# seqan/sahara

Hardware: AMD Instinct MI355X
Metric: reads/s at k=2 edit, 10M×100bp vs 3Gbp index; achieved HBM GB/s (higher is better)
Workload: dtype u32; 1 GPU; C3: k=2 lev, 10000000x100bp reads (+RC) per GPU vs 3 Gbp 24-record index, h2-k2; reads_per_gpu=10000000, read_len=100, errors=2, ref_len=3000000000, records=24, generator=h2-k2, searches=3, parallelism=replicated-index x1 (query shards), hits_total=25990613, build_id=362c7fb006402490

## Files before the change

sahara_amd/csrc/pass.cpp:

```cpp
#include <algorithm>
#include <cstdlib>
#include <chrono>
#include <thread>

#include <sys/prctl.h>

#include "ctx.h"

namespace sahara {

DeviceIndex& partOf(Ctx* c, uint32_t p) { return p == 0 ? c->I : c->more.at(p - 1); }

void run(Ctx* c, bool count) {
    if (c->more.empty()) return runOne(c, count);
    if (c->rounds.size() > 1) throw Error("a pass of several rounds needs a single-part index");
    const ScopeExit routeBack([c, route = c->sk.route] { c->sk.route = route; });
    c->sk.route = HitRoute::Device;
    sahara_stats T{};
    uint64_t total = 0;
    const auto t0 = std::chrono::steady_clock::now();
    for (uint32_t p = 0; p <= c->more.size(); ++p) {
        if (p) std::swap(c->I, c->more[p - 1]);
        {
            const ScopeExit partBack([c, p] {
// ... 54 lines not shown
    S.stage_ms = c->stageMs;
    c->stats = S;
}

const sahara_hit* Ctx::wholeHits() {
    if (outStale) {
        if (out.cap < nout) out.growKeeping(nout, out.cap, st);
        uint64_t b0 = 0;
        for (size_t b = 0; b < batchEnd.size(); b0 = batchEnd[b], ++b)
            if (batchDirect[b])
                launchExpandRecs(outRecs.ptr + b0, batchEnd[b] - b0, batchQ0[b], I.dRecStarts.ptr,
                                 (uint32_t)I.recStarts.size(), out.ptr + b0, st);
        SH_HIP(hipStreamSynchronize(st));
        outStale = false;
    }
    return out.ptr;
}

void initWorkCaps(Ctx* c, uint64_t maxBatch, const PassKnobs& k) {
    if (c->hitCap == 0) c->hitCap = k.hitCap ? k.hitCap : firstWorkCap(maxBatch);
    if (c->taskCap == 0) c->taskCap = k.taskCap ? k.taskCap : firstWorkCap(maxBatch);
}

void reserveSlot(Ctx* c, Ctx::Slot& sl) {
    sl.hits.reserve((size_t)c->hitCap + 1);
    sl.rank.reserve((size_t)c->hitCap + 1);
    sl.tasks.reserve((size_t)c->taskCap);
}

void reserveLocate(Ctx* c, uint64_t maxBatch, uint64_t nslots) {
    c->qoff.reserve(maxBatch + 1);
    c->big.reserve(maxBatch);
    c->huge.reserve(maxBatch);
    for (uint64_t i = 0; i < nslots; ++i) c->slot[i].qcnt.reserve(maxBatch + 1);
}

void growCap(uint32_t& cap, uint32_t seen) {
    const uint64_t want = (uint64_t)seen + seen / 4 + 1024;
    if (want >= (1ull << 32) - 2) throw Error("a work buffer would exceed 2^32 entries in one batch");
    cap = std::max<uint32_t>(cap, (uint32_t)want);
}

static void waitSleepy(hipEvent_t e, uint32_t pollUs) {
    if (!pollUs) {
        SH_HIP(hipEventSynchronize(e));
        return;
    }
    for (;;) {
        const hipError_t r = hipEventQuery(e);
        if (r == hipSuccess) return;
        if (r != hipErrorNotReady) SH_HIP(r);
        std::this_thread::sleep_for(std::chrono::microseconds(pollUs));
    }
}

static PassPlan makePlan(Ctx* c, bool count, bool redo) {
    PassPlan P;
    P.k = readPassKnobs(c->verify);
    const PassKnobs& k = P.k;
    const bool serial = P.serial = redo || !k.pipeline;
    P.count = count;
    P.rounds = (uint32_t)c->rounds.size();
    const WorstRound worst = worstRound(c->rounds);
    if (worst.nsearch != c->nsearch || worst.maxErr != c->maxErr) throw Error("staged rounds do not match their plan");
    const uint32_t sigma = c->I.sigma;
    P.fmLds = fmLdsBytes(c->nsearch, c->m, k.fmLdsDepth);
    const int fullBpc = searchBlocksPerCU(sigma, c->edit, P.fmLds);
    int bpc = fullBpc;
    P.maxBatch = maxBatchOf(k.batch, c->sk.streaming, c->nsearch, c->sk.route == HitRoute::Records);
    const uint64_t batchesHere = (c->npat + P.maxBatch - 1) / P.maxBatch;
    if (!serial && batchesHere > 1 && c->verify) bpc = 1;
    if (k.fmBpc) bpc = (int)std::max<long>(1, std::min<long>(fullBpc, *k.fmBpc));
    P.blocks = (uint32_t)(c->numCU * bpc);
    P.firstBlocks = k.fmBpc ? P.blocks : (uint32_t)(c->numCU * fullBpc);
    P.stackLevels = P.stackCap = fmStackCap(c->maxErr, sigma);

    P.tx = textGeometry(c->m, c->maxErr, c->patBlocks, c->nsearch);
    const bool textFits = text3Blocks(c->I.n) * 16 <= 0xFFFFFF00ull &&
                          P.maxBatch * c->patBlocks * 16 <= 0xFFFFFF00ull;
    P.textShape = textShapeOf(P.tx.winBlocks, c->patBlocks, P.tx.exactWindow);
    auto textAlone = [&] { return textBlocksPerCU(sigma, c->edit, count, P.textShape, P.tx.lds); };
    int tbpc = c->verify && c->m <= 2047 && P.tx.lds <= 160 * 1024 && textFits ? textAlone() : 0;
    if (!serial && batchesHere > 1) tbpc = std::min(tbpc, 3);
    if (k.textBpc && tbpc > 0) tbpc = (int)std::max<long>(1, std::min<long>(textAlone(), *k.textBpc));
    if (k.dump)
        std::fprintf(stderr, "text geometry: shape %d lds %zu blocks/CU %d (alone %d) serial %d\n", P.textShape, P.tx.lds,
                     tbpc, textAlone(), (int)serial);
    P.textBpc = tbpc;
    P.textBlocks = (uint32_t)(c->numCU * std::max(tbpc, 1));
    P.split = tbpc > 0 ? k.split : 0u;
    P.toText = P.split >= 1 && k.seedTasks ? 1u : 0u;
    const bool chunkSeeds = c->sk.streaming && !serial && P.split && k.chunkSeeds;
    P.early = !serial && P.split && (batchesHere > 1 || chunkSeeds) && P.rounds == 1;
    P.chunked0 = P.early && chunkSeeds;
    P.sleepy = c->sk.streaming && !serial;
    P.probe = count && k.dump;
    P.bstart = batchStarts(c->npat, P.maxBatch, k.rampHead, k.rampTail, serial);
    return P;
}

static SearchArgs searchArgs(Ctx* c, const PassPlan& P, Ctx::Slot& sl, uint64_t b, uint32_t r) {
    const uint64_t q0 = P.bstart[b];
    const Ctx::Round& R = c->rounds[r];
    SearchArgs a{};
    a.occF = c->I.occF.ptr;
    a.occR = c->I.occR.ptr;
    for (int i = 0; i < 8; ++i) a.C[i] = (uint32_t)c->I.C[i];
    a.n = (uint32_t)c->I.n;
    a.pats = c->pats.ptr + q0 * c->patWords;
    a.patWords = c->patWords;
    a.m = c->m;
    a.nsearch = R.nsearch;
    a.nitems = (uint32_t)((P.bstart[b + 1] - q0) * R.nsearch);
    a.seeds = sl.seeds.ptr;
    a.seedItem = sl.seedItem.ptr;
    a.seedCount = sl.small.ptr + kSwSeedCount;
    a.scheme = c->scheme.ptr + R.schemeAt;
    a.work = sl.queues.ptr + kQueueSeeds;
    a.hitCount = sl.small.ptr + kSwHitCount;
    a.flags = sl.small.ptr + kSwFlags;
    a.filled = sl.small.ptr + kSwFilled;
    a.taskCount = sl.small.ptr + kSwTaskCount;
    a.stack = c->stack.ptr;
    a.stackCap = P.stackCap;
    a.stackLevels = P.stackLevels;
    a.stealAt = P.k.fmStealAt;
    a.hits = sl.hits.ptr;
    a.hitCap = c->hitCap;
    a.counters = c->counters.ptr;
    a.tasks = sl.tasks.ptr;
    a.taskCap = c->taskCap;
    a.split = P.split;
    a.ldsDepth = P.k.fmLdsDepth;
    a.qcnt = sl.qcnt.ptr;
    a.rank = sl.rank.ptr;
    return a;
}

static SeedArgs seedArgs(Ctx* c, const PassPlan& P, Ctx::Slot& sl, uint64_t b, uint32_t r) {
    const Ctx::Round& R = c->rounds[r];
    SeedArgs sd{};
    sd.pats = c->pats.ptr + P.bstart[b] * c->patWords;
    sd.patWords = c->patWords;
    sd.nsearch = R.nsearch;
    sd.nitems = (uint32_t)((P.bstart[b + 1] - P.bstart[b]) * R.nsearch);
    sd.n = (uint32_t)c->I.n;
    sd.kmer = c->verify && c->I.kmerK ? c->I.kmer.ptr : nullptr;
    sd.kmerK = c->I.kmerK;
    sd.kmerPos = c->I.kmerPos && P.k.kmerPos ? 1u : 0u;
    sd.kmerStart = c->kmerStart.ptr + R.kmerAt;
    sd.seeds = sl.seeds.ptr;
    sd.seedItem = sl.seedItem.ptr;
    sd.seedCount = sl.small.ptr + kSwSeedCount;
    sd.m = c->m;
    sd.toText = P.toText;
    sd.tasks = sl.tasks.ptr;
    sd.taskCap = c->taskCap;
    sd.taskCount = sl.small.ptr + kSwTaskCount;
    sd.flags = sl.small.ptr + kSwFlags;
    sd.counters = P.count ? c->counters.ptr : nullptr;
    sd.skip = r ? sl.qcnt.ptr : nullptr;
    return sd;
}

static TextBatchArgs textArgs(Ctx* c, const PassPlan& P, Ctx::Slot& sl, uint64_t b, uint32_t r) {
    const uint64_t q0 = P.bstart[b];
    const Ctx::Round& R = c->rounds[r];
    TextBatchArgs t{};
    t.sa = c->I.saFull.ptr;
    t.text3 = c->I.text3.ptr;
    t.pats3 = c->pats3.ptr + q0 * c->patBlocks;
    t.patBlocks = c->patBlocks;
    t.text3Bytes = (uint32_t)std::min<uint64_t>(text3Blocks(c->I.n) * 16, 0xFFFFFF00ull);
    t.pats3Bytes = (uint32_t)std::min<uint64_t>((P.bstart[b + 1] - q0) * c->patBlocks * 16, 0xFFFFFF00ull);
    t.m = c->m;
    t.nsearch = R.nsearch;
    t.table = reinterpret_cast<const uint2*>(c->cover.ptr + R.coverAt);
    t.tasks = sl.tasks.ptr;
    t.taskCount = sl.small.ptr + kSwTaskCount;
    t.taskBegin = r ? sl.small.ptr + kSwRoundTasks : nullptr;
    t.taskCap = c->taskCap;
    t.work = sl.queues.ptr + kQueueSeedTasks;
    t.hits = sl.hits.ptr;
    t.hitCap = c->hitCap;
    t.hitCount = sl.small.ptr + kSwHitCount;
    t.filled = sl.small.ptr + kSwFilled;
    t.flags = sl.small.ptr + kSwFlags;
    t.counters = c->counters.ptr;
    t.winBlocks = P.tx.winBlocks;
    t.exactWindow = P.tx.exactWindow ? 1u : 0u;
    t.stackCap = P.tx.textStack;
    t.tableWords = P.tx.tableWords;
    t.steps = P.k.textSteps;
    t.refillAt = P.k.refillAt;
    t.stealAt = P.k.stealAt;
    t.qcnt = sl.qcnt.ptr;
    t.rank = sl.rank.ptr;
    t.probe = P.probe ? 1u : 0u;
    t.isFirst = b == 0 && r == 0 ? 1u : 0u;
    return t;
}

enum : uint32_t { kLocFlags = 2, kLocSegCounts = 4 };

static LocateArgs locateArgs(Ctx* c, Ctx::Slot& sl, uint64_t nhits) {
    LocateArgs la{};
    la.hits = sl.hits.ptr;
    la.nhits = nhits;
    la.qoff = c->qoff.ptr;
    la.rank = sl.rank.ptr;
    la.occF = c->I.occF.ptr;
    for (int i = 0; i < 8; ++i) la.C[i] = (uint32_t)c->I.C[i];
    la.samples = c->I.samples.ptr;
    la.rate = c->I.rate;
    la.keys = c->k0.ptr;
    la.flags = c->small.ptr + kLocFlags;
    la.counters = c->counters.ptr + kCtLfSteps;
    la.sa = c->I.saFull.ptr;
    la.useSA = c->locateSA ? 1u : 0u;
    return la;
}

struct Pass {
    Ctx* c;
    const PassPlan& P;
    sahara_stats& S;
    bool& overflow;
    hipStream_t sA, sB, sC, sD;
    uint32_t seenTask = 0, seenHit = 0;

    Ctx::Slot& slotOf(uint64_t b) const { return c->slot[b % Ctx::kSlots]; }

    void resetSlot(Ctx::Slot& sl, hipStream_t s) {
        SH_HIP(hipMemsetAsync(sl.small.ptr, 0, kSlotWords * sizeof(uint32_t), s));
        SH_HIP(hipMemsetAsync(sl.queues.ptr, 0, kQueuesWords * sizeof(uint32_t), s));
        SH_HIP(hipEventRecord(sl.free, s));
    }
    void freeSlot(Ctx::Slot& sl, hipStream_t s) { SH_HIP(hipEventRecord(sl.free, s)); }

    void seedTasksDone(Ctx::Slot& sl) {
        SH_HIP(hipMemcpyAsync(sl.small.ptr + kSwSeedTasks, sl.small.ptr + kSwTaskCount, 4, hipMemcpyDeviceToDevice, sD));
    }

    struct RoundEv {
        hipEvent_t fmStart, seedDone, fmBegin, fmDone, textStart, textDone;
    };
    RoundEv eventsOf(Ctx::Slot& sl, uint32_t r) const {
        if (r + 1 == P.rounds) return {sl.fmStart, sl.seedDone, sl.fmBegin, sl.fmDone, sl.textStart, sl.textDone};
        Ctx::Slot::RoundEvents& e = sl.earlier[r];
        return {e.fmStart, e.seedDone, e.fmBegin, e.fmDone, e.textStart, e.textDone};
    }

    void issueFM(uint64_t b, uint32_t r) {
        Ctx::Slot& sl = slotOf(b);
        const std::vector<uint64_t>& bstart = P.bstart;
        const RoundEv ev = eventsOf(sl, r);
        const uint32_t nitems = (uint32_t)((bstart[b + 1] - bstart[b]) * c->rounds[r].nsearch);
        if (r == 0) {
            reserveSlot(c, sl);
            SH_HIP(hipStreamWaitEvent(sA, sl.free, 0));
            const uint32_t most = (uint32_t)((bstart[b + 1] - bstart[b]) * c->nsearch);
            sl.seeds.reserve(most);
            sl.seedItem.reserve(most);
        }
        const SearchArgs a = searchArgs(c, P, sl, b, r);
        SeedArgs sd = seedArgs(c, P, sl, b, r);
        if (r == 0) {
            SH_HIP(hipStreamWaitEvent(sD, sl.free, 0));
        } else {
            SH_HIP(hipStreamWaitEvent(sD, eventsOf(sl, r - 1).textDone, 0));
            launchRoundReset(sl.small.ptr, sl.queues.ptr, sD);
        }
        auto seeds = [&](uint32_t i0, uint32_t i1) {
            sd.itemBegin = i0;
            sd.nitems = i1;
            launchSeeds(sd, c->I.sigma, std::max<uint32_t>(1, std::min<uint32_t>((i1 - i0 + 1023) / 1024, (uint32_t)c->numCU * 8)), sD);
// ... 359 lines not shown
```

sahara_amd/csrc/search.hip:

```cpp

#include <hip/hip_runtime.h>

#include <cstring>
#include <type_traits>

#include <rocprim/rocprim.hpp>

#include "search.h"

namespace sahara {
namespace {

#if defined(__HIP_DEVICE_COMPILE__)
#define GLOB(T, p) ((__attribute__((address_space(1))) T*)(p))
#else
#define GLOB(T, p) ((T*)(p))
#endif
typedef uint32_t U32x4 __attribute__((ext_vector_type(4)));
__device__ __forceinline__ uint4 loadGlobal4(const uint4* p) {
    const U32x4 v = *GLOB(const U32x4, p);
    return make_uint4(v.x, v.y, v.z, v.w);
}

__device__ __forceinline__ uint32_t pairSwap(uint32_t v) {
// ... 445 lines not shown
            lo = right ? cur.y : cur.x;
            hi = lo + cur.z;
            needA = matchOK || misOK || delOK;
            needB = needA && (hi >> 6) != (lo >> 6);
        }

        const uint64_t ownA = (uint64_t)(right ? a.occR : a.occF) + (uint64_t)(lo >> 6) * 64u;
        const uint64_t ownB = (uint64_t)(right ? a.occR : a.occF) + (uint64_t)(hi >> 6) * 64u;
        uint32_t ca[5], cb[5];
        uint64_t pa[3], pb[3];
        fetchLinePair(ownA, needA, odd, ca, pa);
        fetchLinePair(ownB, needB, odd, cb, pb);

        if (have) {
            if (COUNT) ++cNodes;
            uint32_t occ[SIGMA], fx[SIGMA], fy[SIGMA];
#pragma unroll
            for (int c = 0; c < SIGMA; ++c) occ[c] = fx[c] = fy[c] = 0;
            if (needA) {
                if (!needB) {
#pragma unroll
                    for (int i = 0; i < 5; ++i) cb[i] = ca[i];
                    pb[0] = pa[0]; pb[1] = pa[1]; pb[2] = pa[2];
                }
                if (COUNT) { ++cRank; cLines += needB ? 2 : 1; }
                const uint64_t ml = lowMask(lo & 63u), mh = lowMask(hi & 63u);
                uint32_t sum = 0, base[SIGMA];
#pragma unroll
                for (int c = 1; c < SIGMA; ++c) {
                    const uint32_t rl = ca[c - 1] + (uint32_t)__popcll(symMask(pa, c) & ml);
                    const uint32_t rh = cb[c - 1] + (uint32_t)__popcll(symMask(pb, c) & mh);
                    occ[c] = rh - rl;
                    base[c] = a.C[c] + rl;
                    sum += occ[c];
                }
                uint32_t acc = (right ? cur.x : cur.y) + (cur.z - sum);
#pragma unroll
                for (int c = 1; c < SIGMA; ++c) {
                    fx[c] = right ? acc : base[c];
                    fy[c] = right ? base[c] : acc;
                    acc += occ[c];
                }
            }
            const uint32_t dl = metaDelta(cur.w);
            auto mk = [&](int c, uint32_t kind) -> uint4 {
                uint32_t f = 0, g = 0, o = 0;
#pragma unroll
                for (int s = 1; s < SIGMA; ++s)
                    if (s == c) { f = fx[s]; g = fy[s]; o = occ[s]; }
                return make_uint4(f, g, o, childMeta(pos, e, lastL, lastR, right, dl, kind));
            };
            auto push = [&](const uint4& v) {
                if (sp - bot < a.stackCap) {
                    stackPut(sp, v);
                    ++sp;
                } else {
                    atomicOr(a.flags, kFlagStack);
                }
            };
            const uint4 ins = make_uint4(cur.x, cur.y, cur.z, childMeta(pos, e, lastL, lastR, right, dl, 3));
            uint4 next = make_uint4(0, 0, 0, 0);
            have = expandChildren<SIGMA>(occ, cq, matchOK, misOK, delOK, insOK, ins, mk, push, next);
            cur = next;
        }
    }
    hitSlots.close(lane, a.hits, a.hitCap);
    taskSlots.close(lane, a.tasks, a.taskCap);
    if (filled) atomicAdd(a.filled, filled);
    if (COUNT) {
        atomicAdd(a.counters + kCtNodes, (unsigned long long)cNodes);
        atomicAdd(a.counters + kCtRankNodes, (unsigned long long)cRank);
        atomicAdd(a.counters + kCtExtLines, (unsigned long long)cLines);
        atomicAdd(a.counters + kCtTextTasks, (unsigned long long)cTasks);
        if (cIter) atomicAdd(a.counters + kCtFmIter, (unsigned long long)cIter);
    }
}




constexpr uint32_t kRun = 32;
constexpr uint32_t kRunMask = 0xFFFFFFFFu;
constexpr uint32_t kChain = 25;
__device__ __forceinline__ uint32_t onesR(uint32_t n) {
    return n >= kRun ? kRunMask : (1u << n) - 1u;
}
__device__ __forceinline__ uint32_t beyondR(uint32_t n) { return kRunMask & ~onesR(n); }
__device__ __forceinline__ uint32_t run7(uint32_t m) {
    const uint32_t m2 = m & (m >> 1), m4 = m2 & (m2 >> 2);
    return m4 & (m2 >> 4) & (m >> 6);
}
struct Planes { uint32_t b0, b1, b2; };
__device__ __forceinline__ uint32_t eqm(const Planes& p, const Planes& t) {
    return ~((p.b0 ^ t.b0) | (p.b1 ^ t.b1) | (p.b2 ^ t.b2));
}
__device__ __forceinline__ Planes shr1(const Planes& p) { return {p.b0 >> 1, p.b1 >> 1, p.b2 >> 1}; }
__device__ __forceinline__ Planes shr2(const Planes& p) { return {p.b0 >> 2, p.b1 >> 2, p.b2 >> 2}; }
__device__ __forceinline__ uint32_t read32(const uint32_t* A, int o, uint32_t b) {
    const int i = o >> 5;
    return __builtin_amdgcn_alignbit(A[(3 * i + 3 + (int)b) * 256], A[(3 * i + (int)b) * 256], (uint32_t)o & 31u);
}
__device__ __forceinline__ Planes chain32(const uint32_t* A, uint32_t o, bool fwd) {
    const int off = (int)o - (fwd ? 0 : 32);
    Planes r;
    uint32_t v[3];
#pragma unroll
    for (uint32_t b = 0; b < 3; ++b) {
        const uint32_t w = read32(A, off, b);
        v[b] = fwd ? w : __builtin_bitreverse32(w);
    }
    r.b0 = v[0]; r.b1 = v[1]; r.b2 = v[2];
    return r;
}

__device__ __forceinline__ __amdgpu_buffer_rsrc_t bufferOf(const void* base, uint32_t bytes) {
    return __builtin_amdgcn_make_buffer_rsrc(const_cast<void*>(base), (short)0, (int)bytes, 0x00020000);
}
constexpr uint32_t kBufOOB = 0xFFFFFFFFu;

__device__ __forceinline__ void copyBlocks(uint32_t* DA, __amdgpu_buffer_rsrc_t RA, uint32_t offA, uint32_t na,
                                           uint32_t* DB, __amdgpu_buffer_rsrc_t RB, uint32_t offB, uint32_t nb) {
    const uint32_t n = max(na, nb);
    for (uint32_t c = 0; c < n; c += 8) {
        decltype(__builtin_amdgcn_raw_buffer_load_b128(RA, 0u, 0, 0)) va[8], vb[8];
#pragma unroll
        for (uint32_t i = 0; i < 8; ++i) {
            const uint32_t j = c + i;
            va[i] = __builtin_amdgcn_raw_buffer_load_b128(RA, j < na ? offA + 16u * j : kBufOOB, 0, 0);
            vb[i] = __builtin_amdgcn_raw_buffer_load_b128(RB, j < nb ? offB + 16u * j : kBufOOB, 0, 0);
        }
#pragma unroll
        for (uint32_t i = 0; i < 8; ++i) {
            const uint32_t j = c + i;
            if (j < na) { uint32_t* D = DA + 3u * j * 256u; D[0] = va[i][0]; D[256] = va[i][1]; D[512] = va[i][2]; }
            if (j < nb) { uint32_t* D = DB + 3u * j * 256u; D[0] = vb[i][0]; D[256] = vb[i][1]; D[512] = vb[i][2]; }
        }
    }
}

__device__ __forceinline__ void copyBlocksShifted(uint32_t* DA, __amdgpu_buffer_rsrc_t RA, uint32_t offA, uint32_t sh,
                                                  uint32_t na, uint32_t* DB, __amdgpu_buffer_rsrc_t RB, uint32_t offB,
                                                  uint32_t nb) {
    decltype(__builtin_amdgcn_raw_buffer_load_b128(RA, 0u, 0, 0)) va[8], vb[8];
#pragma unroll
    for (uint32_t j = 0; j < 8; ++j) {
        va[j] = __builtin_amdgcn_raw_buffer_load_b128(RA, j <= na ? offA + 16u * j : kBufOOB, 0, 0);
        vb[j] = __builtin_amdgcn_raw_buffer_load_b128(RB, j < nb ? offB + 16u * j : kBufOOB, 0, 0);
    }
#pragma unroll
    for (uint32_t j = 0; j < 7; ++j)
        if (j < na) {
            uint32_t* D = DA + 3u * j * 256u;
            D[0] = __builtin_amdgcn_alignbit(va[j + 1][0], va[j][0], sh);
            D[256] = __builtin_amdgcn_alignbit(va[j + 1][1], va[j][1], sh);
            D[512] = __builtin_amdgcn_alignbit(va[j + 1][2], va[j][2], sh);
        }
#pragma unroll
    for (uint32_t j = 0; j < 8; ++j)
        if (j < nb) { uint32_t* D = DB + 3u * j * 256u; D[0] = vb[j][0]; D[256] = vb[j][1]; D[512] = vb[j][2]; }
}

struct TextShape { uint32_t win, pat; bool exact; };
__host__ __device__ constexpr TextShape textShape(int shape) {
    return shape == 1 ? TextShape{4, 4, true} : shape == 2 ? TextShape{9, 8, false} : TextShape{0, 0, false};
}


template <int SIGMA, bool EDIT, bool COUNT, int SHAPE = 0>
__global__ __launch_bounds__(256) void kSearchTextBatch(TextBatchArgs a) {
    extern __shared__ uint32_t lds[];
    uint2* SC = reinterpret_cast<uint2*>(lds);
    uint32_t* slot = lds + a.tableWords;
    for (uint32_t i = threadIdx.x; i < a.nsearch * a.m; i += blockDim.x) SC[i] = a.table[i];
    __syncthreads();
// ... 125 lines not shown
            const uint32_t nI = (uint32_t)__popcll(I), nD = (uint32_t)__popcll(D);
            if (nI >= a.stealAt && nD) {
                const uint32_t n = min(nI, nD);
                const uint32_t r = (uint32_t)__popcll(I & ltMask);
                uint32_t donor = 0, rr = r;
                uint64_t dm = D;
#pragma unroll
                for (uint32_t w = 32; w; w >>= 1) {
                    const uint32_t c = (uint32_t)__popcll(dm & ((1ull << w) - 1ull));
                    if (rr >= c) { rr -= c; dm >>= w; donor += w; }
                }
                const bool takes = thief && r < n;
                donor = takes ? donor : lane;
                const uint32_t dPid = __shfl(pid, donor), dWb = __shfl(wb, donor), dBase = __shfl(sBase, donor);
                const uint32_t dTid = (threadIdx.x & ~63u) | donor;
                if (takes) {
                    const uint32_t* src = slot + dTid;
                    uint32_t* dst = slot + threadIdx.x;
                    for (uint32_t k = 0; k < 3u * (winBlocks + patBlocks); ++k) dst[k * 256u] = src[k * 256u];
                    const uint2 node = reinterpret_cast<const uint2*>(slot + 3u * (winBlocks + patBlocks) * 256u)[dTid];
                    cur = node;
                    pid = dPid;
                    wb = dWb;
                    sBase = dBase;
                    have = true;
                    if (COUNT) ++cSteal;
                }
                __builtin_amdgcn_fence(__ATOMIC_ACQ_REL, "wavefront");
                __builtin_amdgcn_wave_barrier();
                const bool gives = ((D >> lane) & 1ull) && (uint32_t)__popcll(D & ltMask) < n;
                if (gives) {
                    for (uint32_t d = 1; d < sp; ++d) stackPut(d - 1u, stackGet(d));
                    --sp;
                }
            }
        }
        if (!__any(have || sp > 0 || (!exhausted && (!qDone || haveNext || qNext < qEnd)))) break;
        if (kProbe && a.probe) {
            if (qDone && lane == 0 && wDrain[threadIdx.x >> 6] == 0) wDrain[threadIdx.x >> 6] = wall_clock64();
            const uint32_t act = (uint32_t)__popcll(__ballot(have || sp > 0));
            if (qDone) { ++pIterPost; pActPost += act; } else { ++pIterPre; pActPre += act; }
            pw1 = wall_clock64();
        }
        if (COUNT) {
            const uint64_t act = __ballot(have || sp > 0);
            if (lane == 0) { ++tIter; tActive += (uint64_t)__popcll(act); tRefill += refill ? 1u : 0u; }
            const uint64_t t1 = clock64();
            cyRefill += t1 - t0;
            t0 = t1;
        }

        bool leaf = false;
        uint32_t leafStart = 0, leafE = 0;
        for (uint32_t step = 0; step < a.steps; ++step) {
            const bool pop = !have && !leaf && sp > 0;
            const uint2 top = stackGet(pop ? sp - 1u : 0u);
            if (pop) { cur = top; --sp; have = true; }
            const bool live = have && !leaf;
            if (!__any(live)) break;

            const uint32_t pos = cur.y & 0xFFFFu;
            const uint32_t xo = cur.x & 0xFFFFu, yo = cur.x >> 16;
            const uint32_t e = (cur.y >> 16) & 0xFu;
            const uint32_t lastL = (cur.y >> 20) & 3u, lastR = (cur.y >> 22) & 3u;
            const uint2 tab = SC[sBase + min(pos, m - 1u)];
            const uint32_t t0 = tab.x;
            const uint32_t q0 = t0 & 0xFFFFu, lb0 = (t0 >> 16) & 0xFu, ub0 = (t0 >> 20) & 0xFu;
            const bool r0 = (t0 >> 24) & 1u;
            const uint32_t run0 = t0 >> 25, same0 = (tab.y >> 24) & 0x7Fu;

            const Planes P16 = chain32(P, r0 ? q0 : q0 + 1u, r0);
            const Planes T16 = chain32(W, r0 ? yo : xo, r0);
            const uint32_t avail = r0 ? (winLen > yo ? winLen - yo : 0u) : xo;
            const uint32_t VT = onesR(avail);
            const uint32_t E0 = eqm(P16, T16) & VT;
            const uint32_t ED = eqm(P16, shr1(T16)) & (VT >> 1);
            const uint32_t EI = eqm(shr1(P16), T16) & VT;
            const uint32_t TZ = (T16.b0 | T16.b1 | T16.b2) & VT;

            const bool atLeaf = live && pos == m;
            const bool node = live && pos < m;
            const bool forced = e == ub0;
            const bool kidsF = e + 1u == ub0;
            const bool mOK = lb0 <= e && e <= ub0;
            const bool misOK = lb0 <= e + 1u && e + 1u <= ub0;
            const uint32_t side = r0 ? lastR : lastL;
            const uint32_t B = forced ? min(run0, kRun)
                                      : (kidsF ? max(1u, min(min(same0, run0 - 1u), kChain)) : 1u);
            const uint32_t miss = ~E0 & kRunMask;
            const uint32_t L = mOK ? min(B, miss ? (uint32_t)__builtin_ctz(miss) : kRun) : 0u;

            const uint32_t NN = L < B ? L + 1u : B;
            const uint32_t nodesM = node && !forced ? onesR(NN) : 0u;
            const uint32_t first = 1u;
            uint32_t Dm = EDIT ? (nodesM & TZ) : 0u;
            if (pos == 0u || side == OP_I) Dm &= ~first;
            uint32_t Im = EDIT && misOK ? nodesM : 0u;
            if (side == OP_D) Im &= ~first;
            bool Sx = node && !forced && L < B && misOK && ((TZ & ~E0) >> L) & 1u;
            const uint32_t bR = beyondR(run0), bR1 = beyondR(run0 - 1u);
            const uint32_t R7E0 = run7(E0 | bR), R7ED = run7(ED | bR), R7EI = run7(EI | bR1);
            if (kidsF) {
                Dm &= R7ED;
                Im &= R7EI;
                Sx = Sx && ((R7E0 >> (L + 1u)) & 1u);
            }
            if (EDIT && node && e + 2u == ub0) {
                const uint32_t ED2 = eqm(P16, shr2(T16)) & (VT >> 2);
                const uint32_t EI2 = eqm(shr2(P16), T16) & VT;
                const uint32_t bR2 = run0 >= 2u ? beyondR(run0 - 2u) : kRunMask;
                const uint32_t R7ED2 = run7(ED2 | bR), R7EI2 = run7(EI2 | bR2);
                const uint32_t I2after = (R7E0 >> 1) & ~1u;
                constexpr uint32_t kLim = kRun - 9u;
                if (Dm & first) {
                    const uint32_t LD = (uint32_t)__builtin_ctz(~ED);
                    const bool keep = LD >= run0 || LD > kLim || ((R7ED >> (LD + 1u)) & 1u) ||
                                      ((R7ED2 | I2after) & onesR(LD + 1u)) != 0u;
                    if (!keep) Dm &= ~first;
                }
                if (Im & first) {
                    const uint32_t LI = ~EI ? (uint32_t)__builtin_ctz(~EI) : kRun;
                    const bool keep = LI + 1u >= run0 || LI > kLim || ((R7EI >> (LI + 1u)) & 1u) ||
                                      ((I2after | R7EI2) & onesR(LI + 1u)) != 0u;
                    if (!keep) Im &= ~first;
                }
                if (Sx) {
                    const uint32_t rest = ~E0 & ~1u;
                    const uint32_t LS = rest ? (uint32_t)__builtin_ctz(rest) : kRun;
                    Sx = LS >= run0 || LS > kLim || ((R7E0 >> (LS + 1u)) & 1u) ||
                         ((R7ED | R7EI) & ~1u & onesR(LS + 1u)) != 0u;
                }
            }
            const bool contM = node && L >= B;
            uint32_t nSurv = (uint32_t)__popc(Dm) + (uint32_t)__popc(Im) + (Sx ? 1u : 0u);
            uint32_t Bc = B;
            if (nSurv && sp + nSurv + (contM ? 1u : 0u) - 1u > 2u * e + 4u) {
                Bc = 1u;
                Dm &= first;
                Im &= first;
                Sx = Sx && L == 0u;
                nSurv = (uint32_t)__popc(Dm) + (uint32_t)__popc(Im) + (Sx ? 1u : 0u);
            }
            const bool contM1 = node && L >= Bc;
            bad = bad || (node && nSurv && sp + nSurv + (contM1 ? 1u : 0u) - 1u > a.stackCap);

            const int extMul = r0 ? 65536 : -1;
            auto extend = [&](uint32_t span, uint32_t n) -> uint32_t { return span + (uint32_t)((int)n * extMul); };
            const uint32_t shMine = r0 ? 22u : 20u, shOther = r0 ? 20u : 22u;
            const uint32_t otherKept = pos ? (r0 ? lastL : lastR) : (uint32_t)OP_MS;
            auto metaAt = [&](uint32_t i, uint32_t op, uint32_t k) -> uint32_t {
                const uint32_t mine = k ? (uint32_t)OP_MS : op;
                const uint32_t other = (pos == 0u && i == 0u) ? op : otherKept;
                return (mine << shMine) | (other << shOther);
            };
            const uint32_t e1 = (e + 1u) << 16;
            const uint32_t kEnd = kidsF ? run0 : 0u;
            const uint2 cM = make_uint2(extend(cur.x, Bc), (pos + Bc) | (e << 16) | metaAt(Bc, OP_MS, 0u));
            if (nSurv) {
                uint32_t spw = sp;
                uint2 pend = cM;
                bool hasPend = contM1;
                uint64_t sv = (uint64_t)Dm | ((uint64_t)Im << 32) | (Sx ? 1ull << 63 : 0ull);
                while (sv) {
                    const uint32_t j = (uint32_t)__builtin_ctzll(sv);
                    sv &= sv - 1ull;
                    const bool isS = j == 63u, isD = j < 32u, isI = !isD && !isS;
                    const uint32_t i = isS ? L : (j & 31u);
                    const uint32_t ii = i + (isD ? 0u : 1u);
                    const uint32_t k = ii < kEnd ? min(kEnd - ii, 7u) : 0u;
                    const uint32_t op = isD ? (uint32_t)OP_D : (isI ? (uint32_t)OP_I : (uint32_t)OP_MS);
                    const uint2 v = make_uint2(extend(cur.x, i + k + (isI ? 0u : 1u)), (pos + ii + k) | e1 | metaAt(i, op, k));
                    if (hasPend) stackPut(min(spw++, a.stackCap - 1u), pend);
                    pend = v;
                    hasPend = true;
                }
                sp = min(spw, a.stackCap);
                cur = pend;
            } else if (node && contM1) {
                cur = cM;
            }

            if (atLeaf) { leaf = true; leafStart = xo; leafE = e; }
            have = live ? node && (nSurv || contM1) : have;
            if (COUNT) {
                cNodes += forced ? 0u : (node ? NN : 0u);
                cCmp += (node && forced) ? 1u : 0u;
                cSteps += node ? 1u : 0u;
            }
        }
        if (COUNT) {
            const uint64_t t1 = clock64();
            cyStep += t1 - t0;
            t0 = t1;
        }
        {
            uint32_t s;
            if (hitSlots.take(leaf, lane, ltMask, a.hitCount, s) && leaf) {
                if (s < a.hitCap) {
                    a.hits[s] = make_uint4(pid, wb + leafStart, 1u, leafE | kPosKnown);
                    if (rankSlot != ~0u) a.rank[rankSlot] = rankVal;
                    rankVal = atomicAdd(a.qcnt + pid, 1u);
                    rankSlot = s;
                } else {
                    atomicOr(a.flags, kFlagHits);
                }
                ++filled;
            }
        }
        if (COUNT) cyEmit += clock64() - t0;
        if (kProbe && a.probe) {
            const uint64_t pw2 = wall_clock64();
            if (qDone) { pwPostA += pw1 - pw0; pwPostB += pw2 - pw1; }
            else { pwPreA += pw1 - pw0; pwPreB += pw2 - pw1; }
        }
    }
    if (kProbe && a.probe && a.isFirst && lane == 0) {
        const uint64_t wEnd = wall_clock64(), w0 = wBorn[threadIdx.x >> 6], wd = wDrain[threadIdx.x >> 6];
        atomicMin(a.counters + kCtBornMin, (unsigned long long)w0);
        atomicMax(a.counters + kCtBornMax, (unsigned long long)w0);
        atomicMax(a.counters + kCtEndMax, (unsigned long long)wEnd);
        atomicAdd(a.counters + kCtLifeSum, (unsigned long long)(wEnd - w0));
        atomicMin(a.counters + kCtEndMin, (unsigned long long)wEnd);
        if (wd) {
// ... 994 lines not shown
```

sahara_amd/csrc/pass_plan.h:

```cpp
#pragma once
#include <algorithm>
#include <cstdint>
#include <cstdlib>
#include <optional>
#include <vector>

namespace sahara {

constexpr uint32_t kTextTableMin = 3u * 256u;

inline std::vector<uint64_t> parseRamp(const char* e) {
    std::vector<uint64_t> v;
    for (const char* p = e; p && *p;) {
        char* end = nullptr;
        const unsigned long long x = std::strtoull(p, &end, 10);
        if (end == p) break;
        if (x) v.push_back(x);
        p = (*end == ',' || *end == ':') ? end + 1 : end;
    }
    return v;
}

struct PassKnobs {
    bool pipeline, dump, chunkSeeds, kmerPos, seedTasks;
    uint32_t fmLdsDepth, fmStealAt, stealAt, split, textSteps, refillAt, pollUs;
    uint32_t hitCap, taskCap;
    unsigned long timerSlackNs;
    std::optional<long> batch, fmBpc, textBpc;
    std::vector<uint64_t> rampHead, rampTail;
};

inline PassKnobs readPassKnobs(bool verify) {
    auto num = [](const char* name) -> std::optional<long> {
        const char* e = std::getenv(name);
        return e ? std::optional<long>(std::atol(e)) : std::nullopt;
    };
    auto within = [](long lo, long v, long hi) { return std::max(lo, std::min(hi, v)); };
    PassKnobs k{};
    k.pipeline = num("SAHARA_PIPELINE").value_or(1) != 0;
    k.dump = std::getenv("SAHARA_DUMP_COUNTERS") != nullptr;
    k.fmLdsDepth = (uint32_t)within(0, num("SAHARA_FM_LDS_DEPTH").value_or(verify ? 0 : 4), 8);
    k.fmStealAt = (uint32_t)within(0, num("SAHARA_FM_STEAL_AT").value_or(verify ? 0 : 8), 64);
    k.stealAt = (uint32_t)within(0, num("SAHARA_STEAL_AT").value_or(8), 64);
    k.split = (uint32_t)std::max(0L, num("SAHARA_SPLIT").value_or(1));
    k.textSteps = (uint32_t)std::max(1L, num("SAHARA_TEXT_STEPS").value_or(2));
    k.refillAt = (uint32_t)within(1, num("SAHARA_REFILL_AT").value_or(8), 64);
    k.chunkSeeds = num("SAHARA_CHUNK_SEEDS").value_or(1) != 0;
    k.kmerPos = num("SAHARA_KMER_POS").value_or(1) != 0;
    k.seedTasks = num("SAHARA_SEED_TASKS").value_or(1) != 0;
    k.pollUs = (uint32_t)std::max(0L, num("SAHARA_POLL_US").value_or(20));
    k.timerSlackNs = (unsigned long)std::max(0L, num("SAHARA_TIMER_SLACK_NS").value_or(1000));
    if (auto v = num("SAHARA_HITCAP")) k.hitCap = (uint32_t)std::max(1L, *v);
    if (auto v = num("SAHARA_TASKCAP")) k.taskCap = (uint32_t)std::max(1L, *v);
    k.batch = num("SAHARA_BATCH");
    k.fmBpc = num("SAHARA_FM_BPC");
    k.textBpc = num("SAHARA_TEXT_BPC");
    k.rampHead = parseRamp(std::getenv("SAHARA_RAMP"));
    k.rampTail = parseRamp(std::getenv("SAHARA_RAMP_END"));
    return k;
}

inline uint64_t maxBatchOf(std::optional<long> batch, bool streaming, uint32_t nsearch, bool compactRecs) {
    const uint64_t most = (1ull << 31) / nsearch;
    uint64_t mb = std::min<uint64_t>(streaming ? 1ull << 21 : 1ull << 22, most);
    if (batch) mb = std::max<uint64_t>(1, std::min<uint64_t>(most, (uint64_t)*batch));
    return compactRecs ? std::min<uint64_t>(mb, 1ull << 27) : mb;
}

inline uint32_t firstWorkCap(uint64_t maxBatch) {
    return (uint32_t)std::min<uint64_t>(std::max<uint64_t>(1u << 20, 8 * maxBatch), 1u << 30);
}

inline std::vector<uint64_t> batchStarts(uint64_t npat, uint64_t maxBatch, std::vector<uint64_t> head,
                                         std::vector<uint64_t> tail, bool serial) {
    std::vector<uint64_t> bstart{0};
    uint64_t edges = 0;
    for (auto& x : head) edges += x = std::min(x, maxBatch);
    for (auto& x : tail) edges += x = std::min(x, maxBatch);
    if (serial || npat < edges + maxBatch) head.clear(), tail.clear(), edges = 0;
    for (uint64_t x : head) bstart.push_back(bstart.back() + x);
    const uint64_t mid = npat - edges, q0 = bstart.back(), nmid = (mid + maxBatch - 1) / maxBatch;
    for (uint64_t i = 1; i <= nmid; ++i) bstart.push_back(q0 + mid * i / nmid);
    for (uint64_t x : tail) bstart.push_back(bstart.back() + x);
    return bstart;
}

inline size_t fmLdsBytes(uint32_t nsearch, uint32_t m, uint32_t ldsDepth) {
    return (size_t)((nsearch * m + 3u) & ~3u) * 4 + (size_t)ldsDepth * 256 * 16;
}
inline uint32_t fmStackCap(uint32_t maxErr, uint32_t sigma) { return std::max<uint32_t>(maxErr, 1) * (2 * sigma - 2) + 2; }

struct TextGeometry {
    bool exactWindow;
    uint32_t winBlocks, textStack, tableWords;
    size_t lds;
};
inline TextGeometry textGeometry(uint32_t m, uint32_t maxErr, uint32_t patBlocks, uint32_t nsearch) {
    TextGeometry g{};
    const uint32_t exactBlocks = (m + 2 * maxErr + 31) / 32;
    g.exactWindow = exactBlocks + 1 <= 8 && patBlocks <= 8;
    g.winBlocks = g.exactWindow ? exactBlocks : (m + 2 * maxErr + 31 + 31) / 32;
    g.textStack = 2 * maxErr + 2;
    g.tableWords = std::max<uint32_t>(2 * nsearch * m, kTextTableMin);
    g.lds = (size_t)g.tableWords * 4 + (size_t)256 * (3 * (g.winBlocks + patBlocks) + 2 * g.textStack) * 4;
    return g;
}

struct WorstRound {
    uint32_t nsearch = 0, maxErr = 0;
};
template <typename Rounds>
inline WorstRound worstRound(const Rounds& rounds) {
    WorstRound w;
    for (const auto& r : rounds) {
        w.nsearch = std::max(w.nsearch, r.nsearch);
        w.maxErr = std::max(w.maxErr, r.maxErr);
    }
    return w;
}

struct PassPlan {
    PassKnobs k;
    bool count = false, serial = false;
    uint64_t maxBatch = 0;
    std::vector<uint64_t> bstart;
    size_t fmLds = 0;
    uint32_t blocks = 0, firstBlocks = 0, stackCap = 0, stackLevels = 0;
    TextGeometry tx{};
// ... 10 lines not shown
```

sahara_amd/csrc/search.h:

```cpp
#pragma once
#include <hip/hip_runtime.h>

#include <cstddef>
#include <cstdint>

#include "../../include/sahara_hip.h"
#include "device_index.h"

namespace sahara {

struct SearchArgs {
    const OccLine* occF;
    const OccLine* occR;
    uint32_t C[8];
    uint32_t n;
    const uint32_t* pats;
    uint32_t patWords;
    uint32_t m;
    uint32_t nsearch;
    uint32_t nitems;
    const uint4* seeds;
    const uint32_t* seedItem;
    const uint32_t* seedCount;
    const uint32_t* scheme;
// ... 33 lines not shown
    uint32_t* seedCount;
    uint32_t m;
    uint32_t toText;
    uint4* tasks;
    uint32_t taskCap;
    uint32_t* taskCount;
    uint32_t* flags;
    unsigned long long* counters;
    const uint32_t* skip;
};

enum SlotWord : uint32_t {
    kSwRoundTasks = 0,
    kSwHitCount = 1, kSwFlags = 2, kSwFilled = 3, kSwTaskCount = 4,
    kSwSeedTasks = 5,
    kSwSeedCount = 6, kSlotWords = 8
};
enum Flag : uint32_t {
    kFlagStack = 1,
    kFlagHits = 2,
    kFlagLocate = 4,
    kFlagTasks = 8,
    kFlagTextStack = 16
};
constexpr uint32_t kQueueWords = 256;
enum QueueAt : uint32_t { kQueueSeeds = 0, kQueueSeedTasks = kQueueWords, kQueueFmTasks = 2 * kQueueWords,
                         kQueuesWords = 3 * kQueueWords };
struct BatchRecord {
    uint32_t slot[7];
    uint32_t locateFlags;
    uint64_t rows;
    uint32_t nbig, nhuge;
    uint64_t kept;
    uint32_t pad[2];
};
static_assert(sizeof(BatchRecord) == 64 && offsetof(BatchRecord, slot) == 0 &&
              offsetof(BatchRecord, locateFlags) == 4 * 7 && offsetof(BatchRecord, rows) == 4 * kSlotWords &&
              offsetof(BatchRecord, nbig) == 4 * 10 && offsetof(BatchRecord, nhuge) == 4 * 11 &&
              offsetof(BatchRecord, kept) == 4 * 12, "BatchRecord is what kBatchTotals and limitBatch write");

constexpr uint32_t kCounters = 56;
enum Counter : uint32_t {
    kCtNodes = 0, kCtRankNodes = 1, kCtExtLines = 2, kCtLfSteps = 3, kCtDigest = 4, kCtTextNodes = 5,
    kCtTextTasks = 6, kCtFmIter = 7, kCtTextIter = 8, kCtTextActive = 9, kCtTextRefills = 10,
    kCtCyRefill = 11, kCtCyStep = 12, kCtCyEmit = 13,
    kCtCompareSteps = 14, kCtTextSteps = 15,
    kCtPosTasks = 16,
    kCtBestSkipped = 17,
    kCtDryRun = 30, kCtDryWaves = 31,
    kCtBornMin = 33, kCtBornMax = 34, kCtEndMax = 35, kCtLifeSum = 36, kCtEndMin = 37,
    kCtDryMin = 38, kCtDryMax = 39,
    kCtIterPre = 40, kCtActPre = 41, kCtIterPost = 42, kCtActPost = 43,
    kCtStolen = 45,
    kCtWallPreRefill = 46, kCtWallPreStep = 47, kCtWallPostRefill = 48, kCtWallPostStep = 49
};
constexpr uint32_t kTaskPos = 0x80000000u;

struct TextBatchArgs {
    const uint32_t* sa;
    const uint4* text3;
    const uint4* pats3;
    uint32_t patBlocks;
    uint32_t text3Bytes;
    uint32_t pats3Bytes;
    uint32_t m;
    uint32_t nsearch;
    const uint2* table;
    const uint4* tasks;
    const uint32_t* taskCount;
    const uint32_t* taskBegin;
    uint32_t taskCap;
    uint32_t* work;
    uint4* hits;
    uint32_t hitCap;
    uint32_t* hitCount;
    uint32_t* filled;
    uint32_t* flags;
    unsigned long long* counters;
    uint32_t winBlocks;
    uint32_t exactWindow;
    uint32_t stackCap;
    uint32_t tableWords;
    uint32_t steps;
    uint32_t refillAt;
    uint32_t stealAt;
    uint32_t* qcnt;
    uint32_t* rank;
    uint32_t probe;
    uint32_t isFirst;
};

struct LocateArgs {
    const uint4* hits;
    uint64_t nhits;
    const uint64_t* qoff;
    const uint32_t* rank;
    const OccLine* occF;
    uint32_t C[8];
    const uint32_t* samples;
    uint32_t rate;
    uint64_t* keys;
    uint32_t* flags;
    unsigned long long* counters;
    const uint32_t* sa;
    uint32_t useSA;
};

int searchBlocksPerCU(uint32_t sigma, bool edit, size_t lds);
int textBlocksPerCU(uint32_t sigma, bool edit, bool count, int shape, size_t lds);
int textShapeOf(uint32_t winBlocks, uint32_t patBlocks, bool exactWindow);
void launchTextBatch(const TextBatchArgs& a, uint32_t sigma, bool edit, bool count, uint32_t blocks, size_t lds,
                     hipStream_t st);
void launchSeeds(const SeedArgs& a, uint32_t sigma, uint32_t blocks, hipStream_t st);
void launchRoundReset(uint32_t* small, uint32_t* queues, hipStream_t st);
void launchPackPatterns(const uint8_t* src, uint64_t npat, uint32_t m, uint32_t patWords, uint32_t sigma,
                        uint32_t* dst, uint32_t* bad, hipStream_t st);
void launchUnpackNibbles(const uint8_t* nib, uint8_t* dst, uint64_t n, hipStream_t st);
void launchOffsetSeq(const sahara_hit* in, uint64_t n, uint64_t rec0, sahara_hit* out, hipStream_t st);
uint64_t limitBatch(sahara_hit* out, uint64_t rows, const uint64_t* qoff, uint32_t nq, uint32_t n,
                    DevBuf<uint32_t>& kcnt, DevBuf<uint64_t>& koff, DevBuf<sahara_hit>& buf, DevBuf<char>& tmp,
                    uint64_t* hostKept, hipStream_t st);
struct MergeBufs {
    DevBuf<uint64_t> k0, k1;
    DevBuf<uint32_t> v0, v1;
};
void sortHitsByQid(const sahara_hit* in, uint64_t n, uint64_t nqid, sahara_hit* out, MergeBufs& B, DevBuf<char>& tmp,
                   hipStream_t st);
void launchCompactHits(const sahara_hit* h, uint64_t n, uint64_t qidBase, const uint64_t* starts, uint64_t* out,
                       hipStream_t st, uint32_t maxBlocks = 8192);
void launchPackFrom2(const uint8_t* src, uint32_t so, const uint32_t* exc, uint32_t nExc, uint64_t r0, uint64_t p0,
                     uint64_t p1, uint32_t m, bool rc, uint32_t sigma, uint32_t patWords, uint32_t patBlocks,
                     uint32_t* pats, uint4* pats3, hipStream_t st);
void launchInterleaveRC(const uint8_t* reads, uint64_t r0, uint64_t r1, uint32_t m, uint32_t sigma, uint64_t pEnd,
                        uint8_t* pats, hipStream_t st);
void launchSearch(const SearchArgs& a, uint32_t sigma, bool edit, bool count, uint32_t blocks, size_t lds,
                  hipStream_t st);
uint32_t scanTiles(uint32_t nq);
void querySegments(uint32_t* qcnt, uint32_t nq, uint64_t* qoff, uint64_t* partial, uint32_t* big, uint32_t* nbig,
                   uint32_t* huge, uint32_t* nhuge, hipStream_t st);
void launchLocate(const LocateArgs& a, bool count, hipStream_t st);
void launchBatchTotals(uint32_t* small, uint32_t* queues, const uint64_t* rowTotal, uint32_t* segCounts, uint32_t* out,
                       hipStream_t st);
void launchLocateFlagsOut(uint32_t* flags, uint32_t* out, hipStream_t st);
size_t bigSortTempBytes(uint64_t rows, uint32_t nbig);
void sortDecode(uint64_t* k0, uint64_t* k1, uint64_t rows, const uint64_t* qoff, uint32_t nq, const uint32_t* big,
                uint32_t nbig, const uint32_t* huge, uint32_t nhuge, uint64_t qidBase, const uint64_t* starts,
                uint32_t nrec, sahara_hit* out, void* tmp, size_t tmpBytes, hipStream_t st);
void sortCompact(uint64_t* k0, uint64_t* k1, uint64_t rows, const uint64_t* qoff, uint32_t nq, const uint32_t* big,
                 uint32_t nbig, const uint32_t* huge, uint32_t nhuge, uint64_t* out, void* tmp, size_t tmpBytes,
                 hipStream_t st);
void launchExpandRecs(const uint64_t* recs, uint64_t n, uint64_t qidBase, const uint64_t* starts, uint32_t nrec,
                      sahara_hit* out, hipStream_t st);
void launchPackPatterns3(const uint8_t* src, uint64_t npat, uint32_t m, uint32_t patBlocks, uint4* dst,
                         hipStream_t st);
void launchDigest(const sahara_hit* h, uint64_t n, unsigned long long* out, hipStream_t st);
void launchCopyHits(const sahara_hit* h, uint64_t n, uint64_t qidOffset, sahara_hit* dst, hipStream_t st);

}
```

Measured before the change: 928.8 million reads/s.

## Extend run-walk batching to nodes two errors from bound with vectorised pruning

Lets FM-index backtracking nodes that sit two errors below the upper bound advance several characters at once (up to kWalk2), instead of one character per step. Per-position pruning of deletion and insertion branches is generalised from the first position to the whole run with a bitwise prefix-scan (scanDown). When the stack is short on room, the chain length is now sized by binary search so that the surviving branches still fit. A separate tweak caps text-verification blocks per CU at 2 when streaming. The aim is fewer search iterations and stack pushes, paid for with more bit arithmetic per step and a risk of pruning or stack-overflow mistakes.

```diff
diff --git a/sahara_amd/csrc/pass.cpp b/sahara_amd/csrc/pass.cpp
--- a/sahara_amd/csrc/pass.cpp
+++ b/sahara_amd/csrc/pass.cpp
@@ -160,6 +160,7 @@
     auto textAlone = [&] { return textBlocksPerCU(sigma, c->edit, count, P.textShape, P.tx.lds); };
     int tbpc = c->verify && c->m <= 2047 && P.tx.lds <= 160 * 1024 && textFits ? textAlone() : 0;
     if (!serial && batchesHere > 1) tbpc = std::min(tbpc, 3);
+    if (!serial && batchesHere > 1 && c->sk.streaming) tbpc = std::min(tbpc, 2);
     if (k.textBpc && tbpc > 0) tbpc = (int)std::max<long>(1, std::min<long>(textAlone(), *k.textBpc));
     if (k.dump)
         std::fprintf(stderr, "text geometry: shape %d lds %zu blocks/CU %d (alone %d) serial %d\n", P.textShape, P.tx.lds,
diff --git a/sahara_amd/csrc/search.hip b/sahara_amd/csrc/search.hip
--- a/sahara_amd/csrc/search.hip
+++ b/sahara_amd/csrc/search.hip
@@ -551,6 +551,7 @@
 constexpr uint32_t kRun = 32;
 constexpr uint32_t kRunMask = 0xFFFFFFFFu;
 constexpr uint32_t kChain = 25;
+constexpr uint32_t kWalk2 = 23;
 __device__ __forceinline__ uint32_t onesR(uint32_t n) {
     return n >= kRun ? kRunMask : (1u << n) - 1u;
 }
@@ -558,6 +559,14 @@
 __device__ __forceinline__ uint32_t run7(uint32_t m) {
     const uint32_t m2 = m & (m >> 1), m4 = m2 & (m2 >> 2);
     return m4 & (m2 >> 4) & (m >> 6);
+}
+__device__ __forceinline__ uint32_t scanDown(uint32_t A, uint32_t X) {
+#pragma unroll
+    for (uint32_t d = 1; d < 32u; d <<= 1) {
+        A |= X & (A >> d);
+        X &= X >> d;
+    }
+    return A;
 }
 struct Planes { uint32_t b0, b1, b2; };
 __device__ __forceinline__ uint32_t eqm(const Planes& p, const Planes& t) {
@@ -850,11 +859,13 @@
             const bool node = live && pos < m;
             const bool forced = e == ub0;
             const bool kidsF = e + 1u == ub0;
+            const bool kids2 = e + 2u == ub0;
             const bool mOK = lb0 <= e && e <= ub0;
             const bool misOK = lb0 <= e + 1u && e + 1u <= ub0;
             const uint32_t side = r0 ? lastR : lastL;
             const uint32_t B = forced ? min(run0, kRun)
-                                      : (kidsF ? max(1u, min(min(same0, run0 - 1u), kChain)) : 1u);
+                                      : (kidsF || kids2 ? max(1u, min(min(same0, run0 - 1u), kidsF ? kChain : kWalk2))
+                                                        : 1u);
             const uint32_t miss = ~E0 & kRunMask;
             const uint32_t L = mOK ? min(B, miss ? (uint32_t)__builtin_ctz(miss) : kRun) : 0u;
 
@@ -873,30 +884,23 @@
                 Im &= R7EI;
                 Sx = Sx && ((R7E0 >> (L + 1u)) & 1u);
             }
-            if (EDIT && node && e + 2u == ub0) {
+            if (EDIT && node && kids2) {
                 const uint32_t ED2 = eqm(P16, shr2(T16)) & (VT >> 2);
                 const uint32_t EI2 = eqm(shr2(P16), T16) & VT;
                 const uint32_t bR2 = run0 >= 2u ? beyondR(run0 - 2u) : kRunMask;
                 const uint32_t R7ED2 = run7(ED2 | bR), R7EI2 = run7(EI2 | bR2);
-                const uint32_t I2after = (R7E0 >> 1) & ~1u;
                 constexpr uint32_t kLim = kRun - 9u;
-                if (Dm & first) {
-                    const uint32_t LD = (uint32_t)__builtin_ctz(~ED);
-                    const bool keep = LD >= run0 || LD > kLim || ((R7ED >> (LD + 1u)) & 1u) ||
-                                      ((R7ED2 | I2after) & onesR(LD + 1u)) != 0u;
-                    if (!keep) Dm &= ~first;
-                }
-                if (Im & first) {
-                    const uint32_t LI = ~EI ? (uint32_t)__builtin_ctz(~EI) : kRun;
-                    const bool keep = LI + 1u >= run0 || LI > kLim || ((R7EI >> (LI + 1u)) & 1u) ||
-                                      ((I2after | R7EI2) & onesR(LI + 1u)) != 0u;
-                    if (!keep) Im &= ~first;
-                }
+                const uint32_t back0 = R7E0 >> 1;
+                const uint32_t AD = R7ED2 | (~ED & (R7ED >> 1)) | beyondR(min(run0, kLim + 1u));
+                Dm &= AD | (ED & (scanDown(AD | back0, ED) >> 1));
+                const uint32_t AI = R7EI2 | (~EI & (R7EI >> 1)) | beyondR(min(run0 - 1u, kLim + 1u));
+                Im &= AI | (EI & (scanDown(AI | back0, EI) >> 1));
                 if (Sx) {
-                    const uint32_t rest = ~E0 & ~1u;
+                    const uint32_t from = beyondR(L + 1u);
+                    const uint32_t rest = ~E0 & from;
                     const uint32_t LS = rest ? (uint32_t)__builtin_ctz(rest) : kRun;
                     Sx = LS >= run0 || LS > kLim || ((R7E0 >> (LS + 1u)) & 1u) ||
-                         ((R7ED | R7EI) & ~1u & onesR(LS + 1u)) != 0u;
+                         ((R7ED | R7EI) & from & onesR(LS + 1u)) != 0u;
                 }
             }
             const bool contM = node && L >= B;
@@ -904,9 +908,19 @@
             uint32_t Bc = B;
             if (nSurv && sp + nSurv + (contM ? 1u : 0u) - 1u > 2u * e + 4u) {
                 Bc = 1u;
-                Dm &= first;
-                Im &= first;
-                Sx = Sx && L == 0u;
+                if (kids2) {
+                    const uint32_t room = 2u * e + 4u - sp;
+#pragma unroll
+                    for (uint32_t w = 16; w; w >>= 1) {
+                        const uint32_t below = onesR(Bc + w);
+                        if ((uint32_t)__popc(Dm & below) + (uint32_t)__popc(Im & below) <= room) Bc += w;
+                    }
+                    Bc = max(1u, min(Bc, NN - 1u));
+                }
+                const uint32_t below = onesR(Bc);
+                Dm &= below;
+                Im &= below;
+                Sx = Sx && L < Bc;
                 nSurv = (uint32_t)__popc(Dm) + (uint32_t)__popc(Im) + (Sx ? 1u : 0u);
             }
             const bool contM1 = node && L >= Bc;
```

After: 918.7 million reads/s. 1.1% lower.

## Generalize second-to-last-error pruning to all chain positions via bitwise fill

Applied to the files above, without the earlier changes.

Replaces the per-first-node keep checks at the e+2==ub level with a branch-free bit-parallel fill (bitreverse carry propagation) that prunes deletion, insertion and substitution branches at every node in the chain. It also adds a SAHARA_TEXT_WALK knob that lets chains extend at that error level. The walk knob defaults to 1, so chaining there stays as before. The aim is fewer redundant stack pushes and divergent branches in the text-search kernel, at the cost of extra ALU work per step and some risk to correctness.

```diff
diff --git a/sahara_amd/csrc/pass.cpp b/sahara_amd/csrc/pass.cpp
--- a/sahara_amd/csrc/pass.cpp
+++ b/sahara_amd/csrc/pass.cpp
@@ -270,6 +270,7 @@
     t.stackCap = P.tx.textStack;
     t.tableWords = P.tx.tableWords;
     t.steps = P.k.textSteps;
+    t.walk = P.k.textWalk;
     t.refillAt = P.k.refillAt;
     t.stealAt = P.k.stealAt;
     t.qcnt = sl.qcnt.ptr;
diff --git a/sahara_amd/csrc/pass_plan.h b/sahara_amd/csrc/pass_plan.h
--- a/sahara_amd/csrc/pass_plan.h
+++ b/sahara_amd/csrc/pass_plan.h
@@ -23,7 +23,7 @@
 
 struct PassKnobs {
     bool pipeline, dump, chunkSeeds, kmerPos, seedTasks;
-    uint32_t fmLdsDepth, fmStealAt, stealAt, split, textSteps, refillAt, pollUs;
+    uint32_t fmLdsDepth, fmStealAt, stealAt, split, textSteps, textWalk, refillAt, pollUs;
     uint32_t hitCap, taskCap;
     unsigned long timerSlackNs;
     std::optional<long> batch, fmBpc, textBpc;
@@ -44,6 +44,7 @@
     k.stealAt = (uint32_t)within(0, num("SAHARA_STEAL_AT").value_or(8), 64);
     k.split = (uint32_t)std::max(0L, num("SAHARA_SPLIT").value_or(1));
     k.textSteps = (uint32_t)std::max(1L, num("SAHARA_TEXT_STEPS").value_or(2));
+    k.textWalk = (uint32_t)within(1, num("SAHARA_TEXT_WALK").value_or(1), 24);
     k.refillAt = (uint32_t)within(1, num("SAHARA_REFILL_AT").value_or(8), 64);
     k.chunkSeeds = num("SAHARA_CHUNK_SEEDS").value_or(1) != 0;
     k.kmerPos = num("SAHARA_KMER_POS").value_or(1) != 0;
diff --git a/sahara_amd/csrc/search.h b/sahara_amd/csrc/search.h
--- a/sahara_amd/csrc/search.h
+++ b/sahara_amd/csrc/search.h
@@ -139,6 +139,7 @@
     uint32_t stackCap;
     uint32_t tableWords;
     uint32_t steps;
+    uint32_t walk;
     uint32_t refillAt;
     uint32_t stealAt;
     uint32_t* qcnt;
diff --git a/sahara_amd/csrc/search.hip b/sahara_amd/csrc/search.hip
--- a/sahara_amd/csrc/search.hip
+++ b/sahara_amd/csrc/search.hip
@@ -559,6 +559,10 @@
     const uint32_t m2 = m & (m >> 1), m4 = m2 & (m2 >> 2);
     return m4 & (m2 >> 4) & (m >> 6);
 }
+__device__ __forceinline__ uint32_t fillNext(uint32_t Q, uint32_t G) {
+    const uint32_t a = __builtin_bitreverse32(Q | G), b = __builtin_bitreverse32(Q);
+    return __builtin_bitreverse32((a + b) ^ a ^ b);
+}
 struct Planes { uint32_t b0, b1, b2; };
 __device__ __forceinline__ uint32_t eqm(const Planes& p, const Planes& t) {
     return ~((p.b0 ^ t.b0) | (p.b1 ^ t.b1) | (p.b2 ^ t.b2));
@@ -853,8 +857,9 @@
             const bool mOK = lb0 <= e && e <= ub0;
             const bool misOK = lb0 <= e + 1u && e + 1u <= ub0;
             const uint32_t side = r0 ? lastR : lastL;
-            const uint32_t B = forced ? min(run0, kRun)
-                                      : (kidsF ? max(1u, min(min(same0, run0 - 1u), kChain)) : 1u);
+            const bool kidsC = EDIT && e + 2u == ub0;
+            const uint32_t chainMax = kidsF ? kChain : (kidsC ? a.walk : 1u);
+            const uint32_t B = forced ? min(run0, kRun) : max(1u, min(min(same0, run0 - 1u), chainMax));
             const uint32_t miss = ~E0 & kRunMask;
             const uint32_t L = mOK ? min(B, miss ? (uint32_t)__builtin_ctz(miss) : kRun) : 0u;
 
@@ -878,26 +883,15 @@
                 const uint32_t EI2 = eqm(shr2(P16), T16) & VT;
                 const uint32_t bR2 = run0 >= 2u ? beyondR(run0 - 2u) : kRunMask;
                 const uint32_t R7ED2 = run7(ED2 | bR), R7EI2 = run7(EI2 | bR2);
-                const uint32_t I2after = (R7E0 >> 1) & ~1u;
+                const uint32_t back0 = R7E0 >> 1;
                 constexpr uint32_t kLim = kRun - 9u;
-                if (Dm & first) {
-                    const uint32_t LD = (uint32_t)__builtin_ctz(~ED);
-                    const bool keep = LD >= run0 || LD > kLim || ((R7ED >> (LD + 1u)) & 1u) ||
-                                      ((R7ED2 | I2after) & onesR(LD + 1u)) != 0u;
-                    if (!keep) Dm &= ~first;
-                }
-                if (Im & first) {
-                    const uint32_t LI = ~EI ? (uint32_t)__builtin_ctz(~EI) : kRun;
-                    const bool keep = LI + 1u >= run0 || LI > kLim || ((R7EI >> (LI + 1u)) & 1u) ||
-                                      ((I2after | R7EI2) & onesR(LI + 1u)) != 0u;
-                    if (!keep) Im &= ~first;
-                }
-                if (Sx) {
-                    const uint32_t rest = ~E0 & ~1u;
-                    const uint32_t LS = rest ? (uint32_t)__builtin_ctz(rest) : kRun;
-                    Sx = LS >= run0 || LS > kLim || ((R7E0 >> (LS + 1u)) & 1u) ||
-                         ((R7ED | R7EI) & ~1u & onesR(LS + 1u)) != 0u;
-                }
+                const uint32_t out = beyondR(min(run0, kLim + 1u)), outI = beyondR(min(run0 - 1u, kLim + 1u));
+                const uint32_t QD = R7ED2 | (~ED & (R7ED >> 1)) | out;
+                Dm &= QD | (ED & fillNext(QD | back0, ED));
+                const uint32_t QI = R7EI2 | (~EI & (R7EI >> 1)) | outI;
+                Im &= QI | (EI & fillNext(QI | back0, EI));
+                const uint32_t QS = R7ED | R7EI | (~E0 & back0) | out;
+                Sx = Sx && ((fillNext(QS, E0) >> (L & 31u)) & 1u);
             }
             const bool contM = node && L >= B;
             uint32_t nSurv = (uint32_t)__popc(Dm) + (uint32_t)__popc(Im) + (Sx ? 1u : 0u);
```

New measurement: 992.3 million reads/s before, 991.0 million reads/s after, median of 3. Within noise of the previous version (-0.1%).
